# PaddlePaddle/PaddleScience

Measured on AMD Instinct MI355X. Metric: collocation-points/sec (PDE residual+grad), higher is better.
Workload: dtype f32

## Files before the change

### include/ppsci_hip.h

```cpp
#ifndef PPSCI_HIP_H
#define PPSCI_HIP_H

#include <stddef.h>
#include <stdint.h>

#ifdef __cplusplus
extern "C" {
#endif

#define PPSCI_MAX_IN 8
#define PPSCI_MAX_DIRS 4
#define PPSCI_MAX_OUT 8
#define PPSCI_MAX_HIDDEN 16
#define PPSCI_MAX_PROG 128
#define PPSCI_MAX_RES 8
#define PPSCI_MAX_EPARAM 8
#define PPSCI_MAX_AUX 16

enum { PPSCI_OK = 0, PPSCI_E_INVALID = -1, PPSCI_E_UNSUPPORTED = -2, PPSCI_E_LAUNCH = -3 };
enum { PPSCI_ACT_TANH = 0, PPSCI_ACT_SILU = 1, PPSCI_ACT_SIN = 2, PPSCI_ACT_SIGMOID = 3, PPSCI_ACT_COS = 4, PPSCI_ACT_GELU = 5,
       PPSCI_ACT_SWISH = 6, PPSCI_ACT_STAN = 7,
       PPSCI_ACT_RELU = 8, PPSCI_ACT_LEAKY_RELU = 9, PPSCI_ACT_ELU = 10, PPSCI_ACT_SELU = 11, PPSCI_ACT_IDENTITY = 12 };
enum { PPSCI_EMBED_NONE = 0, PPSCI_EMBED_PERIOD = 1,
       PPSCI_EMBED_STREAMS = 2 };
// ... 103 lines not shown

int ppsci_csr_matvec(int64_t rows, int64_t cols, int64_t nnz, const int32_t* row_ptr, const int32_t* col_idx,
                     const float* vals, const float* x, const float* xscale, float alpha, float* y, void* stream);

int ppsci_epilogue_params(const ppsci_epilogue_desc* e, int64_t n_points, const float* const* inputs_host,
                          const float* U, const float* const* aux_host, float* residual_out, float* Ubar,
                          float* loss_partials, const float* eq_params, float* eq_param_partials, void* stream);
int ppsci_epilogue_losses(const ppsci_epilogue_desc* e, int64_t n_points, const float* const* inputs_host,
                          const float* U, const float* const* aux_host, float* residual_out, float* Ubar,
                          float* loss_partials, const float* eq_params, float* eq_param_partials, float* loss_terms,
                          void* counter, void* stream);

int ppsci_causal_weights(int64_t n_points, int n_chunks, float tol, const float* value, const float* label,
                         const float* weight, const float* area, float* chunk_scratch, float* cw, void* stream);

int ppsci_taylor_bwd(const ppsci_mlp_desc* d, const float* params, int64_t n_points,
                     const float* const* inputs_host, const float* Ubar, const void* stash,
                     void* workspace, float* grad_partials, void* stream);
int ppsci_taylor_bwd_ws(const ppsci_mlp_desc* d, const float* params, int64_t n_points,
                        const float* const* inputs_host, const float* Ubar, const void* stash,
                        void* workspace, int64_t workspace_bytes, float* grad_partials, void* stream);

typedef struct ppsci_adam_args {
  float* m;
  float* v;
  float lr, beta1, beta2, eps, grad_scale;
  int64_t step_t;
} ppsci_adam_args;

int64_t ppsci_taylor_step_workspace_bytes(const ppsci_mlp_desc* d, const ppsci_epilogue_desc* e, int64_t n_points);
int ppsci_taylor_step_kind(const ppsci_mlp_desc* d, const ppsci_epilogue_desc* e, int64_t n_points);
void ppsci_set_fused_step(int on);
void ppsci_set_step_tail(int mode);
void ppsci_set_fast_program(int on);
void ppsci_set_static_program(int on);
int ppsci_epilogue_predecode(const ppsci_epilogue_desc* e, uint32_t* out256, int* n_loads);
typedef struct ppsci_step_plan ppsci_step_plan;
ppsci_step_plan* ppsci_taylor_step_plan(const ppsci_mlp_desc* d, const ppsci_epilogue_desc* e, float* params,
                                        int64_t n_points, const float* const* inputs_host, const float* const* aux_host,
                                        float* U, float* Ubar, float* residual_out, void* stash, void* workspace,
                                        int64_t workspace_bytes, float* loss_terms, float* grad);
int ppsci_taylor_step_run(ppsci_step_plan* plan, int accumulate, const ppsci_adam_args* adam, void* stream);
#define PPSCI_STEP_KEEP_FRAGMENTS 1
int ppsci_taylor_step_run_ex(ppsci_step_plan* plan, int accumulate, const ppsci_adam_args* adam, void* stream, int flags);
int ppsci_taylor_step_plan_apply(ppsci_step_plan* plan, const ppsci_adam_args* adam, void* stream);
int ppsci_taylor_step_plan_set_scales(ppsci_step_plan* plan, const ppsci_epilogue_desc* e);
int ppsci_taylor_step_run_main(ppsci_step_plan* plan, void* stream);
void ppsci_taylor_step_plan_free(ppsci_step_plan* plan);
int ppsci_taylor_step_plan_static(const ppsci_step_plan* plan, const char** name);
int ppsci_taylor_step(const ppsci_mlp_desc* d, const ppsci_epilogue_desc* e, float* params, int64_t n_points,
                      const float* const* inputs_host, const float* const* aux_host, float* U, float* Ubar,
                      float* residual_out, void* stash, void* workspace, int64_t workspace_bytes, float* loss_terms,
                      float* grad, int accumulate, const ppsci_adam_args* adam, void* stream);

int ppsci_reduce_rows(const float* partials, int64_t rows, int64_t cols, float* out, int accumulate,
                      void* stream);

int ppsci_adam_step(int64_t n, float* params, const float* grad, float* m, float* v, float lr,
                    float beta1, float beta2, float eps, int64_t step_t, float grad_scale,
                    void* stream);

#define PPSCI_OPT_SGD 0
#define PPSCI_OPT_MOMENTUM 1
#define PPSCI_OPT_RMSPROP 2
#define PPSCI_OPT_ADAMW 3
int ppsci_optim_step(int kind, int64_t n, float* params, const float* grad, float* state1, float* state2,
// ... 299 lines not shown
```

### paddlescience_amd/_lib.py

```python
from __future__ import annotations

import ctypes as C
import os
from typing import List, Optional, Sequence

MAX_IN, MAX_DIRS, MAX_OUT, MAX_HIDDEN, MAX_PROG, MAX_RES, MAX_AUX = 8, 4, 8, 16, 128, 8, 16

ACT = {"tanh": 0, "silu": 1, "sin": 2, "sigmoid": 3, "cos": 4, "gelu": 5, "swish": 6, "stan": 7, "relu": 8, "leaky_relu": 9,
       "elu": 10, "selu": 11, "identity": 12}
PARAM_ACTS = ("swish", "stan")
SIREN_W0 = 30.0
LINEAR_PLAIN, LINEAR_WEIGHT_NORM, LINEAR_RWF, LINEAR_FOURIER, LINEAR_BROADCAST = range(5)
LINEAR_PADDED = 100
EMBED_NONE, EMBED_PERIOD, EMBED_STREAMS = 0, 1, 2

(OP_LD_IN, OP_LD_U, OP_LD_AUX, OP_CONST, OP_ADD, OP_SUB, OP_MUL, OP_DIV, OP_NEG, OP_POW, OP_SIN, OP_COS,
 OP_TANH, OP_EXP, OP_LOG, OP_SQRT, OP_ABS, OP_SINH, OP_COSH, OP_TAN, OP_MAX, OP_MIN, OP_SIGN, OP_HEAVISIDE,
 OP_DETACH, OP_ASIN, OP_ACOS, OP_ATAN, OP_ATAN2, OP_ASINH, OP_ACOSH, OP_ATANH, OP_ERF, OP_LGAMMA, OP_CEIL, OP_FLOOR,
 OP_LD_PARAM, OP_COUNT) = range(38)
MAX_EPARAM = 8
STEP_KEEP_FRAGMENTS = 1


class MlpDesc(C.Structure):
# ... 106 lines not shown
    "ppsci_comm_init": (C.c_int, [C.c_int, C.c_int, C.c_void_p]),
    "ppsci_comm_world_size": (C.c_int, []),
    "ppsci_allreduce_sum": (C.c_int, [C.c_void_p, C.c_int64, C.c_void_p]),
    "ppsci_allgather": (C.c_int, [C.c_void_p, C.c_void_p, C.c_int64, C.c_void_p]),
    "ppsci_comm_destroy": (C.c_int, []),
    "ppsci_param_count": (C.c_int64, [C.POINTER(MlpDesc)]),
    "ppsci_stash_bytes": (C.c_int64, [C.POINTER(MlpDesc), C.c_int64]),
    "ppsci_bwd_partial_rows": (C.c_int64, [C.POINTER(MlpDesc), C.c_int64]),
    "ppsci_bwd_workspace_bytes": (C.c_int64, [C.POINTER(MlpDesc), C.c_int64]),
    "ppsci_epilogue_partial_rows": (C.c_int64, [C.c_int64]),
    "ppsci_taylor_fwd": (C.c_int, [C.POINTER(MlpDesc), C.c_void_p, C.c_int64, C.POINTER(C.c_void_p), C.c_void_p,
                                   C.c_void_p, C.c_void_p]),
    "ppsci_epilogue": (C.c_int, [C.POINTER(EpilogueDesc), C.c_int64, C.POINTER(C.c_void_p), C.c_void_p,
                                 C.POINTER(C.c_void_p), C.c_void_p, C.c_void_p, C.c_void_p, C.c_void_p]),
    "ppsci_epilogue_losses": (C.c_int, [C.POINTER(EpilogueDesc), C.c_int64, C.POINTER(C.c_void_p), C.c_void_p,
                                        C.POINTER(C.c_void_p), C.c_void_p, C.c_void_p, C.c_void_p, C.c_void_p,
                                        C.c_void_p, C.c_void_p, C.c_void_p, C.c_void_p]),
    "ppsci_epilogue_params": (C.c_int, [C.POINTER(EpilogueDesc), C.c_int64, C.POINTER(C.c_void_p), C.c_void_p,
                                        C.POINTER(C.c_void_p), C.c_void_p, C.c_void_p, C.c_void_p, C.c_void_p,
                                        C.c_void_p, C.c_void_p]),
    "ppsci_taylor_bwd": (C.c_int, [C.POINTER(MlpDesc), C.c_void_p, C.c_int64, C.POINTER(C.c_void_p), C.c_void_p,
                                   C.c_void_p, C.c_void_p, C.c_void_p, C.c_void_p]),
    "ppsci_taylor_bwd_ws": (C.c_int, [C.POINTER(MlpDesc), C.c_void_p, C.c_int64, C.POINTER(C.c_void_p), C.c_void_p,
                                      C.c_void_p, C.c_void_p, C.c_int64, C.c_void_p, C.c_void_p]),
    "ppsci_dense_matvec": (C.c_int, [C.c_int64, C.c_int64, C.c_void_p, C.c_void_p, C.c_void_p, C.c_float, C.c_int, C.c_void_p,
                                     C.c_void_p]),
    "ppsci_csr_matvec": (C.c_int, [C.c_int64, C.c_int64, C.c_int64, C.c_void_p, C.c_void_p, C.c_void_p, C.c_void_p, C.c_void_p,
                                   C.c_float, C.c_void_p, C.c_void_p]),
    "ppsci_reduce_rows": (C.c_int, [C.c_void_p, C.c_int64, C.c_int64, C.c_void_p, C.c_int, C.c_void_p]),
    "ppsci_taylor_step_workspace_bytes": (C.c_int64, [C.POINTER(MlpDesc), C.POINTER(EpilogueDesc), C.c_int64]),
    "ppsci_taylor_step_kind": (C.c_int, [C.POINTER(MlpDesc), C.POINTER(EpilogueDesc), C.c_int64]),
    "ppsci_set_fused_step": (None, [C.c_int]),
    "ppsci_set_step_tail": (None, [C.c_int]),
    "ppsci_set_fast_program": (None, [C.c_int]),
    "ppsci_taylor_step_run_ex": (C.c_int, [C.c_void_p, C.c_int, C.POINTER(AdamArgs), C.c_void_p, C.c_int]),
    "ppsci_taylor_step_plan_apply": (C.c_int, [C.c_void_p, C.POINTER(AdamArgs), C.c_void_p]),
    "ppsci_set_static_program": (None, [C.c_int]),
    "ppsci_epilogue_predecode": (C.c_int, [C.POINTER(EpilogueDesc), C.POINTER(C.c_uint32), C.POINTER(C.c_int)]),
    "ppsci_taylor_step_plan_static": (C.c_int, [C.c_void_p, C.POINTER(C.c_char_p)]),
    "ppsci_taylor_step_plan": (C.c_void_p, [C.POINTER(MlpDesc), C.POINTER(EpilogueDesc), C.c_void_p, C.c_int64,
                                            C.POINTER(C.c_void_p), C.POINTER(C.c_void_p), C.c_void_p, C.c_void_p, C.c_void_p,
                                            C.c_void_p, C.c_void_p, C.c_int64, C.c_void_p, C.c_void_p]),
    "ppsci_taylor_step_run": (C.c_int, [C.c_void_p, C.c_int, C.POINTER(AdamArgs), C.c_void_p]),
    "ppsci_taylor_step_plan_set_scales": (C.c_int, [C.c_void_p, C.POINTER(EpilogueDesc)]),
    "ppsci_taylor_step_run_main": (C.c_int, [C.c_void_p, C.c_void_p]),
    "ppsci_taylor_step_plan_free": (None, [C.c_void_p]),
    "ppsci_taylor_step": (C.c_int, [C.POINTER(MlpDesc), C.POINTER(EpilogueDesc), C.c_void_p, C.c_int64, C.POINTER(C.c_void_p),
                                    C.POINTER(C.c_void_p), C.c_void_p, C.c_void_p, C.c_void_p, C.c_void_p, C.c_void_p,
                                    C.c_int64, C.c_void_p, C.c_void_p, C.c_int, C.POINTER(AdamArgs), C.c_void_p]),
    "ppsci_spectral_conv2d_fwd": (C.c_int, [C.POINTER(SpectralDesc), C.c_void_p, C.c_void_p, C.c_void_p, C.c_void_p,
                                            C.c_void_p]),
    "ppsci_spectral_conv2d_bwd": (C.c_int, [C.POINTER(SpectralDesc), C.c_void_p, C.c_void_p, C.c_void_p, C.c_void_p,
                                            C.c_void_p, C.c_void_p, C.c_void_p, C.c_void_p]),
    "ppsci_spectral_conv2d_bwd_real": (C.c_int, [C.POINTER(SpectralDesc), C.c_void_p, C.c_void_p, C.c_void_p, C.c_void_p,
                                                 C.c_void_p, C.c_void_p, C.c_void_p, C.c_float, C.c_int, C.c_void_p]),
    "ppsci_spectral_conv2d_fwd_scaled": (C.c_int, [C.POINTER(SpectralDesc), C.c_void_p, C.c_void_p, C.c_void_p, C.c_void_p,
                                                   C.c_float, C.c_int, C.c_void_p]),
    "ppsci_spectral_conv2d_bwd_real_scaled": (C.c_int, [C.POINTER(SpectralDesc), C.c_void_p, C.c_void_p, C.c_void_p,
                                                        C.c_void_p, C.c_void_p, C.c_void_p, C.c_void_p, C.c_float, C.c_int,
                                                        C.c_float, C.c_int, C.c_void_p]),
    "ppsci_dft2_kept_supported": (C.c_int, [C.c_int] * 4),
    "ppsci_dft2_kept_fwd": (C.c_int, [C.c_int] * 6 + [C.c_void_p] * 3),
    "ppsci_dft2_kept_inv": (C.c_int, [C.c_int] * 6 + [C.c_void_p] * 3),
    "ppsci_dft2_kept_inv_stats": (C.c_int, [C.c_int] * 6 + [C.c_void_p] * 3 + [C.c_int, C.c_void_p, C.c_void_p]),
    "ppsci_fno_tail_fwd_ex": (C.c_int, [C.c_int] * 5 + [C.c_float] + [C.c_void_p] * 9 + [C.c_int] * 5 + [C.c_void_p, C.c_void_p]),
    "ppsci_fno_tail_bwd_ex": (C.c_int, [C.c_int] * 5 + [C.c_void_p] * 13 + [C.c_int] * 4 + [C.c_void_p] * 3),
# ... 210 lines not shown
```

### paddlescience_amd/csrc/ppsci_common.h

```cpp
#pragma once

#include "ppsci_hip.h"

#ifdef PPSCI_EMU
#include "hip_emu.h"
#define PPSCI_LAUNCH(KERNEL, ARGT, grid, block, lds, stream, args)                                   \
  do {                                                                                               \
    ARGT _a = (args);                                                                                \
    emu::launch_named(#KERNEL, emu_dim3{(unsigned)(grid)}, emu_dim3{(unsigned)(block)}, (size_t)(lds), \
                      [](void* p) { KERNEL(*(ARGT*)p); }, &_a);                                      \
  } while (0)
#define PPSCI_SET_MAX_LDS(KERNEL, bytes) (0)
#define PPSCI_LAST_LAUNCH_ERROR() (0)
#define PPSCI_OCCUPANCY(KERNEL, block, lds, out) (*(out) = 2, 0)
#define __builtin_amdgcn_sched_barrier(x) ((void)0)
#define ppsci_block_sync_lds() __syncthreads()
#define ppsci_block_sync_mem() __syncthreads()
#define ppsci_acquire_agent() ((void)0)
#define ppsci_setprio(p) ((void)0)
#define PPSCI_OPAQUE(v) ((void)0)
static inline void ppsci_store_agent(float* p, float v) { *p = v; }
static inline void ppsci_store_agent4(f32x4* p, f32x4 v) { *p = v; }
static inline unsigned ppsci_readlane(unsigned v, int lane) {
  float f;
  std::memcpy(&f, &v, 4);
  const float* buf = emu::wave_publish(f);
  unsigned r;
  std::memcpy(&r, &buf[lane & 63], 4);
  return r;
}
#else
#include <hip/hip_runtime.h>
typedef float f32x4 __attribute__((ext_vector_type(4)));
typedef unsigned u32x2 __attribute__((ext_vector_type(2)));
typedef unsigned u32x4 __attribute__((ext_vector_type(4)));
#define PPSCI_DYN_SMEM(name) extern __shared__ __attribute__((aligned(16))) float name[]
#define PPSCI_OPAQUE(v) asm volatile("" : "+v"(v))
__device__ __forceinline__ unsigned ppsci_cvt_pk_bf16(float a, float b) {
  typedef float f32x2_ __attribute__((ext_vector_type(2)));
  typedef __bf16 bf16x2_ __attribute__((ext_vector_type(2)));
  return __builtin_bit_cast(unsigned, __builtin_convertvector((f32x2_){a, b}, bf16x2_));
}
__device__ __forceinline__ float ppsci_bf16_sub_lo(unsigned h, float x) {
  typedef __bf16 bf16x2_ __attribute__((ext_vector_type(2)));
  unsigned k = 0x0000bf80u;
  asm volatile("" : "+s"(k));
  return __builtin_amdgcn_fdot2_f32_bf16(__builtin_bit_cast(bf16x2_, h), __builtin_bit_cast(bf16x2_, k), x, false);
}
__device__ __forceinline__ float ppsci_bf16_sub_hi(unsigned h, float x) {
  typedef __bf16 bf16x2_ __attribute__((ext_vector_type(2)));
  unsigned k = 0xbf800000u;
  asm volatile("" : "+s"(k));
  return __builtin_amdgcn_fdot2_f32_bf16(__builtin_bit_cast(bf16x2_, h), __builtin_bit_cast(bf16x2_, k), x, false);
}
__device__ __forceinline__ f32x4 ppsci_xdl32(u32x2 a_lo, u32x2 a_hi, u32x2 b_lo, u32x2 b_hi, f32x4 c) {
  typedef __bf16 bf16x8_ __attribute__((ext_vector_type(8)));
  const u32x4 a = {a_lo[0], a_lo[1], a_hi[0], a_hi[1]}, b = {b_lo[0], b_lo[1], b_hi[0], b_hi[1]};
  return __builtin_amdgcn_mfma_f32_16x16x32_bf16(__builtin_bit_cast(bf16x8_, a), __builtin_bit_cast(bf16x8_, b), c, 0, 0, 0);
}
__device__ __forceinline__ f32x4 ppsci_xdl32a(u32x4 a, u32x2 b_lo, u32x2 b_hi, f32x4 c) {
  typedef __bf16 bf16x8_ __attribute__((ext_vector_type(8)));
  const u32x4 b = {b_lo[0], b_lo[1], b_hi[0], b_hi[1]};
  return __builtin_amdgcn_mfma_f32_16x16x32_bf16(__builtin_bit_cast(bf16x8_, a), __builtin_bit_cast(bf16x8_, b), c, 0, 0, 0);
}
__device__ __forceinline__ f32x4 ppsci_xdl32aa(u32x4 a, u32x4 b, f32x4 c) {
  typedef __bf16 bf16x8_ __attribute__((ext_vector_type(8)));
  return __builtin_amdgcn_mfma_f32_16x16x32_bf16(__builtin_bit_cast(bf16x8_, a), __builtin_bit_cast(bf16x8_, b), c, 0, 0, 0);
}
__device__ __forceinline__ u32x2 ppsci_lds_read_tr16(const void* p) {
  typedef short s16x4_ __attribute__((ext_vector_type(4)));
  return __builtin_bit_cast(u32x2, __builtin_amdgcn_ds_read_tr16_b64_v4i16((__attribute__((address_space(3))) s16x4_*)p));
}
__device__ __forceinline__ f32x4 ppsci_xdl16(u32x2 a, u32x2 b, f32x4 c) {
  typedef short s16x4_ __attribute__((ext_vector_type(4)));
  return __builtin_amdgcn_mfma_f32_16x16x16bf16_1k(__builtin_bit_cast(s16x4_, a), __builtin_bit_cast(s16x4_, b), c, 0, 0, 0);
}
#define PPSCI_LAUNCH(KERNEL, ARGT, grid, block, lds, stream, args)                                   \
  hipLaunchKernelGGL(KERNEL, dim3(grid), dim3(block), (lds), (hipStream_t)(stream), (args))
#define PPSCI_SET_MAX_LDS(KERNEL, bytes)                                                             \
  ((int)hipFuncSetAttribute((const void*)KERNEL, hipFuncAttributeMaxDynamicSharedMemorySize, (int)(bytes)))
#define PPSCI_LAST_LAUNCH_ERROR() ((int)hipGetLastError())
#define PPSCI_OCCUPANCY(KERNEL, block, lds, out)                                                     \
  ((int)hipOccupancyMaxActiveBlocksPerMultiprocessor((out), (const void*)KERNEL, (block), (size_t)(lds)))
__device__ __forceinline__ void ppsci_wave_sync() {
  __builtin_amdgcn_fence(__ATOMIC_RELEASE, "wavefront", "local");
// ... 88 lines not shown
```

### paddlescience_amd/csrc/taylor_fused.inc

```
#include "taylor_tile.h"
#include "taylor_step_tail.h"
#include "epi_static.h"

#include <stdlib.h>
#include <string.h>
#include <type_traits>

#ifndef PPSCI_FUSED_STATIC
#define PPSCI_FUSED_STATIC 0
#endif
#define PPSCI_FUSED_EPI_SCRATCH ((PPSCI_MAX_RES + PPSCI_MAX_EPARAM) * 16)
#define PPSCI_FUSED_MAX_IN 4
#define PPSCI_FUSED_XJ(x, j) ((j) == 0 ? (x)[0] : ((j) == 1 ? (x)[1] : ((j) == 2 ? (x)[2] : (x)[3])))

#ifdef PPSCI_FUSED_TIMERS
#define PPSCI_FT(k)                                             \
  {                                                             \
    const unsigned long long now_ = __builtin_amdgcn_s_memtime(); \
    tacc[k] += now_ - tlast;                                    \
    tlast = now_;                                               \
  }
#else
#define PPSCI_FT(k)
#endif

#define PPSCI_ABL(n) (((ABL) >> (n)) & 1)
template <int ABL>
__device__ __forceinline__ ppsci_split4 ppsci_fused_split(f32x4 x) {
  if (PPSCI_ABL(6)) {
    ppsci_split4 o;
    o.p[0] = (u32x2){__builtin_bit_cast(unsigned, x[0]), __builtin_bit_cast(unsigned, x[1])};
    o.p[1] = (u32x2){__builtin_bit_cast(unsigned, x[2]), __builtin_bit_cast(unsigned, x[3])};
    o.p[2] = o.p[0];
    return o;
  }
  return ppsci_split(x);
}

#ifdef PPSCI_DBG_DUMP
__device__ float* ppsci_dbg_buf = nullptr;
extern "C" int ppsci_dbg_set(float* p) { return (int)hipMemcpyToSymbol(HIP_SYMBOL(ppsci_dbg_buf), &p, sizeof(p)); }
#define PPSCI_DBG_STRIDE 16384
#endif


static inline long long ppsci_fused_floats(const ppsci_mlp_desc& d, const ppsci_derived& q, int S, int n_instr) {
  const int m = d.d_out, pad4m = ((m + 3) / 4) * 4;
  long long fl = 2LL * ((q.d0 + d.n_hidden + m) * q.HP + pad4m);
  fl += (q.NB + 1) * m * S * PPSCI_TILE;
  fl += q.NB * d.d_raw * PPSCI_TILE;
  fl += (long long)q.NB * m * S * PPSCI_TILE;
  fl += PPSCI_FUSED_EPI_SCRATCH + PPSCI_MAX_RES * PPSCI_TILE;
  fl += 2LL * n_instr * PPSCI_TILE;
  fl += EPI_FAST_WORDS + PPSCI_MAX_RES + PPSCI_MAX_RES * PPSCI_TILE;
  fl += 2LL * S * q.NB * 3 * 64 * 2;
  fl += PPSCI_MAX_DIRS * q.HP;
  return fl;
}

template <int NB, int LH, int N1, int N2, int ACT, bool STATIC, int ABL = 0>
__global__ void __launch_bounds__(64 * NB, 2) taylor_fused_kernel(StepArgs args) {
  constexpr int S = 1 + N1 + N2;
  constexpr int HP = 16 * NB;
  constexpr int W = NB;
  constexpr int L = LH;
  constexpr int NKP = NB / 2;
  static_assert(NB == 4, "one feature block per wave, both k-pairs of a layer's fragments held in registers");
  PPSCI_DYN_SMEM(smem);
  const FwdArgs& a = args.f;
  const int tid = threadIdx.x, nthr = blockDim.x;
  const int lane = tid & 63, wave = __builtin_amdgcn_readfirstlane(tid >> 6);
  const int g = lane >> 4, c = lane & 15;
  const int H = a.d.width, m = a.d.d_out, d0 = a.q.d0, d_raw = a.d.d_raw;
  const int pad4m = ((m + 3) / 4) * 4;
  const int n_instr = args.e.e.n_instr;

  float* W0s = smem;
  float* Bs = W0s + d0 * HP;
  float* WLs = Bs + L * HP;
  float* BLs = WLs + m * HP;
  float* gW0 = BLs + pad4m;
  float* gB = gW0 + d0 * HP;
  float* gWL = gB + L * HP;
  float* gBL = gWL + m * HP;
  float* tin = gBL + pad4m;
  float* uls = tin + W * m * S * PPSCI_TILE;
  float* tinx = uls + m * S * PPSCI_TILE;
  float* red = tinx + W * d_raw * PPSCI_TILE;
  float* ered = red + W * m * S * PPSCI_TILE;
  float* lacc = ered + PPSCI_FUSED_EPI_SCRATCH;
  float* rf = lacc + PPSCI_MAX_RES * PPSCI_TILE;
  unsigned* ftab = (unsigned*)(rf + 2 * n_instr * PPSCI_TILE);
  float* rres = (float*)(ftab + EPI_FAST_WORDS + PPSCI_MAX_RES);
  u32x2* zx = (u32x2*)(rres + PPSCI_MAX_RES * PPSCI_TILE);
  u32x2* hx = zx + S * NB * 3 * 64;
  float* dz0 = (float*)(hx + S * NB * 3 * 64);
  f32x4* zsave = (f32x4*)hx;
  static_assert(L * S * 64 * 16 <= S * NB * 3 * 64 * 8, "zsave must fit into hx");
  constexpr bool VM_REGS_OK = (L - 1) * NB * 64 * 16 <= S * NB * 3 * 64 * 8;
// ... 18 lines not shown
    for (int idx = tid; idx < N1 * HP; idx += nthr) {
      const int i = idx / HP, f = idx - i * HP;
      float acc = 0.f;
      for (int j = 0; j < d_raw; ++j) acc += ((f < H) ? a.params[a.q.offW[0] + j * H + f] : 0.f) * a.d.dirs[i][j];
      dz0[idx] = acc;
    }
  const int nacc_small = (d0 + L + m) * HP + pad4m;
  for (int idx = tid; idx < nacc_small; idx += nthr) gW0[idx] = 0.f;
  for (int idx = tid; idx < PPSCI_MAX_RES * PPSCI_TILE; idx += nthr) lacc[idx] = 0.f;
  if (args.e.fast != nullptr) epi_fast_init(args.e, ftab, rf + (lane & 15), PPSCI_TILE, tid, nthr, wave == 0 && lane < PPSCI_TILE);

  float xr[PPSCI_FUSED_MAX_IN];
  const auto fetch_x = [&](int tile_, float (&dst)[PPSCI_FUSED_MAX_IN]) {
    const long long p_ = (long long)tile_ * PPSCI_TILE + c;
    const bool ok_ = tile_ < a.ntiles && p_ < a.N;
#pragma unroll
    for (int j = 0; j < PPSCI_FUSED_MAX_IN; ++j) dst[j] = (j < d_raw && ok_) ? a.x[j < d_raw ? j : 0][p_] : 0.f;
  };
  fetch_x(a.tile0 + (int)blockIdx.x, xr);
  __syncthreads();
  const int static_id = STATIC ? args.e.static_id : 0;
  float st_cvals = 0.f, st_scales = 0.f;
  if constexpr (STATIC) {
    st_cvals = __builtin_bit_cast(float, ftab[192 + (lane & 63)]);
    st_scales = __builtin_bit_cast(float, ftab[EPI_FAST_WORDS + (lane & (PPSCI_MAX_RES - 1))]);
  }

  f32x4 wacc[L - 1][NB];
#pragma unroll
  for (int l = 0; l < L - 1; ++l)
#pragma unroll
    for (int ib = 0; ib < NB; ++ib) wacc[l][ib] = (f32x4){0.f, 0.f, 0.f, 0.f};

#ifdef PPSCI_FUSED_TIMERS
  if (tid < 16) ((unsigned*)ered)[tid] = 0u;
  unsigned long long tacc[16] = {0, 0, 0, 0, 0, 0, 0, 0, 0, 0, 0, 0, 0, 0, 0, 0};
  unsigned long long tlast = __builtin_amdgcn_s_memtime();
#endif
  for (int it = 0; it < a.iters; ++it) {
    const int tile = a.tile0 + it * (int)gridDim.x + (int)blockIdx.x;
    if (tile >= a.ntiles) break;
    PPSCI_FT(0)
    const float* tx = STATIC ? tinx + wave * (d_raw * PPSCI_TILE) : tinx;
    float* const tinw = STATIC ? tin + wave * (m * S * PPSCI_TILE) : tin;
    float auxv[EPI_STATIC_MAX_AUX];
#pragma unroll
    for (int k = 0; k < EPI_STATIC_MAX_AUX; ++k) auxv[k] = 0.f;
    if (STATIC && args.e.e.n_aux > 0) {
      const long long p_ = (long long)tile * PPSCI_TILE + c;
      const long long pp_ = p_ < a.N ? p_ : 0;
#pragma unroll
      for (int k = 0; k < EPI_STATIC_MAX_AUX; ++k)
        if (k < args.e.e.n_aux) auxv[k] = args.e.aux[k][pp_];
    }
    f32x4 zst[L][S];
    f32x4 h[S];

#pragma unroll
    for (int s = 0; s < S; ++s) h[s] = (f32x4){0.f, 0.f, 0.f, 0.f};
    {
      const long long p = (long long)tile * PPSCI_TILE + c;
      const long long pp = p < a.N ? p : 0;
      const float vm = p < a.N ? 1.f : 0.f;
      int k = 0;
      if (PPSCI_ABL(1)) h[0] += xr[0] * 0.01f;
      if ((STATIC || raw_only) && !PPSCI_ABL(1)) {
// ... 382 lines not shown
          *(f32x4*)&q[(2 * 256 + tid) * 4] = D1;
        }
#endif
        {
          const f32x4 two = {2.f, 2.f, 2.f, 2.f};
          f32x4 accv = D1 * hb[0];
#pragma unroll
          for (int i = 0; i < N1; ++i) {
            const f32x4 zi = zst[l][1 + i];
            const f32x4 hbi = hb[1 + i];
            f32x4 zbi = D1 * hbi;
            accv += D2 * zi * hbi;
            if (i < N2) {
              const f32x4 zii = zst[l][1 + N1 + i];
              const f32x4 hb2 = hb[1 + N1 + i];
              hb[1 + N1 + i] = D1 * hb2;
              zbi += two * D2 * zi * hb2;
              accv += (D3 * zi * zi + D2 * zii) * hb2;
            }
            hb[1 + i] = zbi;
          }
          hb[0] = accv;
        }
        if (zs != 1.f) {
#pragma unroll
          for (int s = 0; s < S; ++s) hb[s] *= zs;
        }
#ifdef PPSCI_DBG_DUMP
        if (ppsci_dbg_buf != nullptr && l == L - 1) {
#pragma unroll
          for (int s = 0; s < S; ++s) *(f32x4*)&ppsci_dbg_buf[(long long)blockIdx.x * PPSCI_DBG_STRIDE + (s * 256 + tid) * 4] = hb[s];
        }
#endif
        if (!PPSCI_ABL(2)) {
          f32x4 sb4;
#pragma unroll
          for (int r = 0; r < 4; ++r) sb4[r] = ppsci_row_sum16_last(hb[0][r]);
#ifdef PPSCI_DBG_DUMP
          if (ppsci_dbg_buf != nullptr && l == L - 1) *(f32x4*)&ppsci_dbg_buf[(long long)blockIdx.x * PPSCI_DBG_STRIDE + 4096 + tid * 4] = sb4;
#endif
          if (c == 15) {
#pragma unroll
            for (int r = 0; r < 4; ++r) atomicAdd(&gB[l * HP + 16 * wave + 4 * g + r], sb4[r]);
          }
        }
        if constexpr (l > 0) {
          __builtin_amdgcn_sched_barrier(0);
#pragma unroll
          for (int kp = 0; kp < NKP; ++kp)
#pragma unroll
            for (int q = 0; q < 3; ++q) Ab[kp][q] = gf[((wave * NKP + kp) * 3 + q) * 64];
          __builtin_amdgcn_sched_barrier(0);
#pragma unroll
          for (int s = 0; s < S; ++s) {
            const ppsci_split4 sp = ppsci_fused_split<ABL>(hb[s]);
#pragma unroll
            for (int q = 0; q < 3; ++q)
              if (!PPSCI_ABL(9) || (sp.p[q][0] == 0x12345u && sp.p[q][1] == 0x54321u)) zx[ppsci_xpair(NB, s, wave, q, xcl)] = sp.p[q];
            __builtin_amdgcn_sched_barrier(0);
          }
        }
      }

      if constexpr (l > 0) {
        __builtin_amdgcn_sched_barrier(0);
        ppsci_block_sync_lds();
        PPSCI_FT(7)
// ... 190 lines not shown
        }
      }
    };
#ifndef PPSCI_FX_NOBWD
    if constexpr (L > 4) bwd_layer(std::integral_constant<int, 4>{});
    if constexpr (L > 3) bwd_layer(std::integral_constant<int, 3>{});
    if constexpr (L > 2) bwd_layer(std::integral_constant<int, 2>{});
    bwd_layer(std::integral_constant<int, 1>{});
#endif
    bwd_layer(std::integral_constant<int, 0>{});

    PPSCI_FT(11)
    PPSCI_FT(12)
  }
#ifdef PPSCI_FUSED_TIMERS
  if (lane == 0 && args.t.external && wave != 1) {
#pragma unroll
    for (int k = 0; k < 16; ++k) args.t.tree[((long long)blockIdx.x * W + wave) * 16 + k] = (float)tacc[k];
    if (wave == 0)
      for (int k = 0; k < 16; ++k) args.t.tree[((long long)blockIdx.x * W + 1) * 16 + k] = (float)((unsigned*)ered)[k];
  }
#endif

  {
    f32x4* dst = args.b.wpart + (long long)blockIdx.x * ((L - 1) * NB * NB * 64) + lane;
#pragma unroll
    for (int l = 0; l < L - 1; ++l)
#pragma unroll
      for (int ib = 0; ib < NB; ++ib) {
        f32x4* const q = &dst[((long long)l * NB * NB + ib * NB + wave) * 64];
        if (args.t.external == 1) *q = wacc[l][ib];
        else ppsci_store_agent4(q, wacc[l][ib]);
      }
  }
  __syncthreads();
  for (int idx = tid; idx < d0 * H; idx += nthr) {
    const int k = idx / H, f = idx - k * H;
    ppsci_store_agent(&prow[idx], gW0[k * HP + f]);
  }
  for (int idx = tid; idx < L * H; idx += nthr) {
    const int l = idx / H, f = idx - l * H;
    ppsci_store_agent(&prow[d0 * H + idx], gB[l * HP + f]);
  }
  for (int idx = tid; idx < H * m; idx += nthr) {
    const int f = idx / m, cc = idx - f * m;
    ppsci_store_agent(&prow[(d0 + L) * H + idx], gWL[cc * HP + f]);
  }
  for (int idx = tid; idx < m; idx += nthr) ppsci_store_agent(&prow[(d0 + L + m) * H + idx], gBL[idx]);
  {
    float lsum[PPSCI_MAX_RES], padj[PPSCI_MAX_EPARAM];
#pragma unroll
    for (int k = 0; k < PPSCI_MAX_RES; ++k) lsum[k] = (wave == 0 && lane < PPSCI_TILE) ? lacc[k * PPSCI_TILE + lane] : 0.f;
#pragma unroll
    for (int k = 0; k < PPSCI_MAX_EPARAM; ++k) padj[k] = 0.f;
    epi_finale<EPI_RF_FUSED>(args.e, ered, lsum, padj);
  }
  if (args.t.external != 1) ppsci_step_tail(args.t, args.b.d, args.b.q, smem);
}

template <int NB, int LH, int N1, int N2>
static int launch_fused(StepArgs& a, void* stream, int launch, int* grid_out) {
  constexpr int S = 1 + N1 + N2;
  if (launch == 2) {
#ifdef PPSCI_ABL_BUILD
    {
      const char* ev = getenv("PPSCI_ABL");
// ... 87 lines not shown
```

### paddlescience_amd/csrc/taylor_fused_silu.hip

```cpp
#define PPSCI_ACT_ID PPSCI_ACT_SILU
#define PPSCI_FUSED_RUN_NAME ppsci_fused_run_silu
#include "taylor_fused.inc"
```

### paddlescience_amd/csrc/taylor_fused_sin.hip

```cpp
#define PPSCI_ACT_ID PPSCI_ACT_SIN
#define PPSCI_FUSED_RUN_NAME ppsci_fused_run_sin
#include "taylor_fused.inc"
```

### paddlescience_amd/csrc/taylor_fused_static_tanh.hip

```cpp
#define PPSCI_ACT_ID PPSCI_ACT_TANH
#define PPSCI_FUSED_STATIC 1
#define PPSCI_FUSED_RUN_NAME ppsci_fused_static_run_tanh
#include "taylor_fused.inc"
```

### paddlescience_amd/csrc/wgrad_reduce.hip

```cpp
#include "taylor_tile.h"

#include <string.h>

struct WRedArgs {
  const float* wpart;
  float* tmp;
  float* row;
  const float* small;
  float* tmp_small;
  int nsmall_rows, psmall, nbs;
  int m, d0;
  ppsci_derived q;
  int L, H, ntiles, nchunks, nb4;
  long long per_tile;
  long long tmp_stride, small_stride, loss_stride;
  ppsci_wred_extras x;
};

__global__ void __launch_bounds__(256) wgrad_reduce1_kernel(WRedArgs a) {
  if ((int)blockIdx.x >= a.nchunks * a.nb4) {
    const int bid = (int)blockIdx.x - a.nchunks * a.nb4;
    const int chunk = bid / a.nbs;
    const int j = (bid - chunk * a.nbs) * 256 + threadIdx.x;
    if (j >= a.psmall) return;
// ... 162 lines not shown
    }
  }
  PPSCI_LAUNCH(wgrad_reduce2_kernel, WRedArgs, (q.P + 255) / 256 + (x.loss_rows != nullptr ? 1 : 0), 256, 0, stream, a);
  int e = PPSCI_LAST_LAUNCH_ERROR();
  if (e != 0) {
    ppsci_set_error("wgrad_reduce2: launch failed (hip error %d)", e);
    return PPSCI_E_LAUNCH;
  }
  return PPSCI_OK;
}

struct WTailArgs {
  const float* rows_w;
  const float* rows_s;
  float* row;
  u32x4* frag;
  ppsci_derived q;
  int L, H, m, d0, nrows, psmall, nblk, nsmall;
  long long per_tile, loss_stride;
  ppsci_wred_extras x;
};

__device__ __forceinline__ float wtail_adam(const ppsci_wred_extras& x, int idx, float gsum) {
  const float g = gsum * x.grad_scale;
  const float mm = x.beta1 * x.m[idx] + (1.f - x.beta1) * g;
  const float vv = x.beta2 * x.v[idx] + (1.f - x.beta2) * g * g;
  x.m[idx] = mm;
  x.v[idx] = vv;
  const float pn = x.p[idx] - x.lr_t * (mm / (sqrtf(vv) + x.eps_t));
  x.p[idx] = pn;
  return pn;
}

__global__ void __launch_bounds__(1024) wgrad_tail_kernel(WTailArgs a) {
  __shared__ f32x4 red[16][64];
  __shared__ float tile[16][17];
  const int tid = threadIdx.x, lane = tid & 63, rg = tid >> 6;
  const int b = blockIdx.x;
  if (b < a.nblk) {
    const long long stride4 = a.per_tile / 4;
    const f32x4* src = (const f32x4*)a.rows_w + (long long)b * 64 + lane;
    f32x4 acc[4];
#pragma unroll
    for (int u = 0; u < 4; ++u) acc[u] = (f32x4){0.f, 0.f, 0.f, 0.f};
#pragma unroll 2
    for (int r0 = rg; r0 < a.nrows; r0 += 64) {
#pragma unroll
      for (int u = 0; u < 4; ++u) {
        const int r = r0 + 16 * u;
        const f32x4 v = __builtin_nontemporal_load(&src[(long long)(r < a.nrows ? r : a.nrows - 1) * stride4]);
        acc[u] += r < a.nrows ? v : (f32x4){0.f, 0.f, 0.f, 0.f};
      }
    }
    red[rg][lane] = (acc[0] + acc[1]) + (acc[2] + acc[3]);
    __syncthreads();
    if (rg != 0) return;
    f32x4 tot = red[0][lane];
#pragma unroll
    for (int w = 1; w < 16; ++w) tot += red[w][lane];
    const int NB = a.q.NB, NKP = NB / 2;
    const int l = b / (NB * NB), blk = b - l * NB * NB, ib = blk / NB, ob = blk - ib * NB;
    const int g = lane >> 4, c = lane & 15;
    const int in0 = 16 * ib + 4 * g, out = 16 * ob + c;
    f32x4 pn = (f32x4){0.f, 0.f, 0.f, 0.f};
#pragma unroll
    for (int r = 0; r < 4; ++r) {
// ... 17 lines not shown
    for (int r = 0; r < 4; ++r) tile[4 * g + r][c] = pn[r];
    ppsci_wave_sync();
    f32x4 pt;
#pragma unroll
    for (int r = 0; r < 4; ++r) pt[r] = tile[c][4 * g + r];
    {
      const ppsci_split4 sp = ppsci_split(pt);
      u32x2* dst = (u32x2*)(a.frag + (long long)(a.L - 1 + l) * per_layer + (long long)((ib * NKP + (ob >> 1)) * 3) * 64 + lane) + (ob & 1);
#pragma unroll
      for (int p = 0; p < 3; ++p) dst[(long long)p * 64 * 2] = sp.p[p];
    }
    return;
  }
  if (b < a.nblk + a.nsmall) {
    float* redf = (float*)red;
    const int ci = (b - a.nblk) * 64 + lane;
    const int cc = ci < a.psmall ? ci : 0;
    float acc[4] = {0.f, 0.f, 0.f, 0.f};
#pragma unroll 2
    for (int r0 = rg; r0 < a.nrows; r0 += 64) {
#pragma unroll
      for (int u = 0; u < 4; ++u) {
        const int r = r0 + 16 * u;
        const float v = a.rows_s[(long long)(r < a.nrows ? r : a.nrows - 1) * a.psmall + cc];
        acc[u] += r < a.nrows ? v : 0.f;
      }
    }
    redf[rg * 64 + lane] = (acc[0] + acc[1]) + (acc[2] + acc[3]);
    __syncthreads();
    if (rg != 0 || ci >= a.psmall) return;
    float v = redf[lane];
#pragma unroll
    for (int w = 1; w < 16; ++w) v += redf[w * 64 + lane];
    const int H = a.H, L = a.L;
    int idx;
    if (ci < a.d0 * H) idx = a.q.offW[0] + ci;
    else if (ci < (a.d0 + L) * H) {
      const int lb = (ci - a.d0 * H) / H;
      idx = a.q.offB[lb] + (ci - a.d0 * H - lb * H);
    } else if (ci < (a.d0 + L + a.m) * H) idx = a.q.offW[L] + (ci - (a.d0 + L) * H);
    else idx = a.q.offB[L] + (ci - (a.d0 + L + a.m) * H);
    if (a.x.accumulate) v += a.row[idx];
    a.row[idx] = v;
    if (a.x.p != nullptr) wtail_adam(a.x, idx, v);
    return;
  }
  float* redf = (float*)red;
  for (int k = 0; k < a.x.n_res; ++k) {
    float v = 0.f;
#pragma unroll 4
    for (int r = tid; r < a.x.loss_nrows; r += 1024) v += a.x.loss_rows[(long long)r * a.loss_stride + k];
#pragma unroll
    for (int off = 32; off >= 1; off >>= 1) v += __shfl_xor(v, off, 64);
    if (lane == 0) redf[rg] = v;
    __syncthreads();
    if (tid == 0) {
      float s = redf[0];
      for (int w = 1; w < 16; ++w) s += redf[w];
      a.x.loss_out[k] = s;
    }
    __syncthreads();
  }
}

int ppsci_wgrad_tail(const ppsci_mlp_desc& d, const ppsci_derived& q, int nrows, const float* rows_w, const float* rows_s,
                     float* row, const ppsci_wred_extras& x, void* frag, void* stream) {
  WTailArgs a;
  memset(&a, 0, sizeof(a));
  a.rows_w = rows_w;
  a.rows_s = rows_s;
  a.row = row;
  a.frag = (u32x4*)frag;
  a.q = q;
  a.L = d.n_hidden;
  a.H = d.width;
  a.m = d.d_out;
  a.d0 = q.d0;
  a.nrows = nrows;
  a.psmall = ppsci_small_params(d, q);
  a.nblk = (d.n_hidden - 1) * q.NB * q.NB;
  a.nsmall = (a.psmall + 63) / 64;
  a.per_tile = (long long)(d.n_hidden - 1) * q.HP * q.HP;
  a.loss_stride = x.n_res;
  a.x = x;
  PPSCI_LAUNCH(wgrad_tail_kernel, WTailArgs, a.nblk + a.nsmall + (x.loss_rows != nullptr ? 1 : 0), 1024, 0, stream, a);
  if (PPSCI_LAST_LAUNCH_ERROR() != 0) {
    ppsci_set_error("wgrad_tail: launch failed");
    return PPSCI_E_LAUNCH;
  }
  return PPSCI_OK;
}
```

Before: 445.1 million.

## Split weight-gradient tail into smaller blocks, accumulate biases per lane, tweak split constants

The weight-gradient tail reduction gets a new 256-thread kernel that gives each 16x16 tile four blocks instead of one 1024-thread block, and this kernel is now the default path. The aim is more parallelism and better occupancy in the tail. Separately, the fused forward kernel keeps per-lane bias-gradient accumulators for small configs and does the 16-lane row sum once at the end rather than every iteration. This trades extra registers for fewer cross-lane reductions. The bf16 split constant is also held in a VGPR for the silu, sin and static-tanh variants, which may change instruction selection and register pressure.

Result: faster. 467.8 million, median of 6 (+5.1%).

```diff
diff --git a/include/ppsci_hip.h b/include/ppsci_hip.h
--- a/include/ppsci_hip.h
+++ b/include/ppsci_hip.h
@@ -159,6 +159,7 @@
 int ppsci_taylor_step_kind(const ppsci_mlp_desc* d, const ppsci_epilogue_desc* e, int64_t n_points);
 void ppsci_set_fused_step(int on);
 void ppsci_set_step_tail(int mode);
+void ppsci_set_tail_split(int n);
 void ppsci_set_fast_program(int on);
 void ppsci_set_static_program(int on);
 int ppsci_epilogue_predecode(const ppsci_epilogue_desc* e, uint32_t* out256, int* n_loads);
diff --git a/paddlescience_amd/_lib.py b/paddlescience_amd/_lib.py
--- a/paddlescience_amd/_lib.py
+++ b/paddlescience_amd/_lib.py
@@ -162,6 +162,7 @@
     "ppsci_taylor_step_kind": (C.c_int, [C.POINTER(MlpDesc), C.POINTER(EpilogueDesc), C.c_int64]),
     "ppsci_set_fused_step": (None, [C.c_int]),
     "ppsci_set_step_tail": (None, [C.c_int]),
+    "ppsci_set_tail_split": (None, [C.c_int]),
     "ppsci_set_fast_program": (None, [C.c_int]),
     "ppsci_taylor_step_run_ex": (C.c_int, [C.c_void_p, C.c_int, C.POINTER(AdamArgs), C.c_void_p, C.c_int]),
     "ppsci_taylor_step_plan_apply": (C.c_int, [C.c_void_p, C.POINTER(AdamArgs), C.c_void_p]),
diff --git a/paddlescience_amd/csrc/ppsci_common.h b/paddlescience_amd/csrc/ppsci_common.h
--- a/paddlescience_amd/csrc/ppsci_common.h
+++ b/paddlescience_amd/csrc/ppsci_common.h
@@ -41,16 +41,21 @@
   typedef __bf16 bf16x2_ __attribute__((ext_vector_type(2)));
   return __builtin_bit_cast(unsigned, __builtin_convertvector((f32x2_){a, b}, bf16x2_));
 }
+#if defined(PPSCI_SPLIT_CONST_VGPR) && PPSCI_SPLIT_CONST_VGPR
+#define PPSCI_SPLIT_CONST_HIDE(k) asm("" : "+v"(k))
+#else
+#define PPSCI_SPLIT_CONST_HIDE(k) asm volatile("" : "+s"(k))
+#endif
 __device__ __forceinline__ float ppsci_bf16_sub_lo(unsigned h, float x) {
   typedef __bf16 bf16x2_ __attribute__((ext_vector_type(2)));
   unsigned k = 0x0000bf80u;
-  asm volatile("" : "+s"(k));
+  PPSCI_SPLIT_CONST_HIDE(k);
   return __builtin_amdgcn_fdot2_f32_bf16(__builtin_bit_cast(bf16x2_, h), __builtin_bit_cast(bf16x2_, k), x, false);
 }
 __device__ __forceinline__ float ppsci_bf16_sub_hi(unsigned h, float x) {
   typedef __bf16 bf16x2_ __attribute__((ext_vector_type(2)));
   unsigned k = 0xbf800000u;
-  asm volatile("" : "+s"(k));
+  PPSCI_SPLIT_CONST_HIDE(k);
   return __builtin_amdgcn_fdot2_f32_bf16(__builtin_bit_cast(bf16x2_, h), __builtin_bit_cast(bf16x2_, k), x, false);
 }
 __device__ __forceinline__ f32x4 ppsci_xdl32(u32x2 a_lo, u32x2 a_hi, u32x2 b_lo, u32x2 b_hi, f32x4 c) {
diff --git a/paddlescience_amd/csrc/taylor_fused.inc b/paddlescience_amd/csrc/taylor_fused.inc
--- a/paddlescience_amd/csrc/taylor_fused.inc
+++ b/paddlescience_amd/csrc/taylor_fused.inc
@@ -8,6 +8,9 @@
 
 #ifndef PPSCI_FUSED_STATIC
 #define PPSCI_FUSED_STATIC 0
+#endif
+#ifndef PPSCI_FUSED_LANE_BIAS
+#define PPSCI_FUSED_LANE_BIAS(L, S, ACT, STATIC) ((L) * ((S) + 1) <= (((STATIC) && (ACT) == PPSCI_ACT_TANH) ? 20 : 12))
 #endif
 #define PPSCI_FUSED_EPI_SCRATCH ((PPSCI_MAX_RES + PPSCI_MAX_EPARAM) * 16)
 #define PPSCI_FUSED_MAX_IN 4
@@ -65,6 +68,7 @@
   constexpr int W = NB;
   constexpr int L = LH;
   constexpr int NKP = NB / 2;
+  constexpr bool LANE_BIAS = PPSCI_FUSED_LANE_BIAS(LH, S, ACT, STATIC);
   static_assert(NB == 4, "one feature block per wave, both k-pairs of a layer's fragments held in registers");
   PPSCI_DYN_SMEM(smem);
   const FwdArgs& a = args.f;
@@ -149,6 +153,10 @@
 #pragma unroll
     for (int ib = 0; ib < NB; ++ib) wacc[l][ib] = (f32x4){0.f, 0.f, 0.f, 0.f};
 
+  f32x4 bacc[LANE_BIAS ? L : 1];
+#pragma unroll
+  for (int l = 0; l < (LANE_BIAS ? L : 1); ++l) bacc[l] = (f32x4){0.f, 0.f, 0.f, 0.f};
+
 #ifdef PPSCI_FUSED_TIMERS
   if (tid < 16) ((unsigned*)ered)[tid] = 0u;
   unsigned long long tacc[16] = {0, 0, 0, 0, 0, 0, 0, 0, 0, 0, 0, 0, 0, 0, 0, 0};
@@ -597,7 +605,9 @@
           for (int s = 0; s < S; ++s) *(f32x4*)&ppsci_dbg_buf[(long long)blockIdx.x * PPSCI_DBG_STRIDE + (s * 256 + tid) * 4] = hb[s];
         }
 #endif
-        if (!PPSCI_ABL(2)) {
+        if constexpr (LANE_BIAS) {
+          if (!PPSCI_ABL(2)) bacc[l] += hb[0];
+        } else if (!PPSCI_ABL(2)) {
           f32x4 sb4;
 #pragma unroll
           for (int r = 0; r < 4; ++r) sb4[r] = ppsci_row_sum16_last(hb[0][r]);
@@ -854,6 +864,15 @@
         if (args.t.external == 1) *q = wacc[l][ib];
         else ppsci_store_agent4(q, wacc[l][ib]);
       }
+  }
+  if constexpr (LANE_BIAS) {
+#pragma unroll
+    for (int l = 0; l < L; ++l) {
+      f32x4 sb4;
+#pragma unroll
+      for (int r = 0; r < 4; ++r) sb4[r] = ppsci_row_sum16_last(bacc[l][r]);
+      if (c == 15) *(f32x4*)&gB[l * HP + 16 * wave + 4 * g] = sb4;
+    }
   }
   __syncthreads();
   for (int idx = tid; idx < d0 * H; idx += nthr) {
diff --git a/paddlescience_amd/csrc/taylor_fused_silu.hip b/paddlescience_amd/csrc/taylor_fused_silu.hip
--- a/paddlescience_amd/csrc/taylor_fused_silu.hip
+++ b/paddlescience_amd/csrc/taylor_fused_silu.hip
@@ -1,3 +1,6 @@
+#ifndef PPSCI_SPLIT_CONST_VGPR
+#define PPSCI_SPLIT_CONST_VGPR 1
+#endif
 #define PPSCI_ACT_ID PPSCI_ACT_SILU
 #define PPSCI_FUSED_RUN_NAME ppsci_fused_run_silu
 #include "taylor_fused.inc"
diff --git a/paddlescience_amd/csrc/taylor_fused_sin.hip b/paddlescience_amd/csrc/taylor_fused_sin.hip
--- a/paddlescience_amd/csrc/taylor_fused_sin.hip
+++ b/paddlescience_amd/csrc/taylor_fused_sin.hip
@@ -1,3 +1,6 @@
+#ifndef PPSCI_SPLIT_CONST_VGPR
+#define PPSCI_SPLIT_CONST_VGPR 1
+#endif
 #define PPSCI_ACT_ID PPSCI_ACT_SIN
 #define PPSCI_FUSED_RUN_NAME ppsci_fused_run_sin
 #include "taylor_fused.inc"
diff --git a/paddlescience_amd/csrc/taylor_fused_static_tanh.hip b/paddlescience_amd/csrc/taylor_fused_static_tanh.hip
--- a/paddlescience_amd/csrc/taylor_fused_static_tanh.hip
+++ b/paddlescience_amd/csrc/taylor_fused_static_tanh.hip
@@ -1,3 +1,6 @@
+#ifndef PPSCI_SPLIT_CONST_VGPR
+#define PPSCI_SPLIT_CONST_VGPR 1
+#endif
 #define PPSCI_ACT_ID PPSCI_ACT_TANH
 #define PPSCI_FUSED_STATIC 1
 #define PPSCI_FUSED_RUN_NAME ppsci_fused_static_run_tanh
diff --git a/paddlescience_amd/csrc/wgrad_reduce.hip b/paddlescience_amd/csrc/wgrad_reduce.hip
--- a/paddlescience_amd/csrc/wgrad_reduce.hip
+++ b/paddlescience_amd/csrc/wgrad_reduce.hip
@@ -218,6 +218,17 @@
   return pn;
 }
 
+__device__ __forceinline__ int wtail_small_index(const WTailArgs& a, int ci) {
+  const int H = a.H, L = a.L;
+  if (ci < a.d0 * H) return a.q.offW[0] + ci;
+  if (ci < (a.d0 + L) * H) {
+    const int lb = (ci - a.d0 * H) / H;
+    return a.q.offB[lb] + (ci - a.d0 * H - lb * H);
+  }
+  if (ci < (a.d0 + L + a.m) * H) return a.q.offW[L] + (ci - (a.d0 + L) * H);
+  return a.q.offB[L] + (ci - (a.d0 + L + a.m) * H);
+}
+
 __global__ void __launch_bounds__(1024) wgrad_tail_kernel(WTailArgs a) {
   __shared__ f32x4 red[16][64];
   __shared__ float tile[16][17];
@@ -301,14 +312,7 @@
     float v = redf[lane];
 #pragma unroll
     for (int w = 1; w < 16; ++w) v += redf[w * 64 + lane];
-    const int H = a.H, L = a.L;
-    int idx;
-    if (ci < a.d0 * H) idx = a.q.offW[0] + ci;
-    else if (ci < (a.d0 + L) * H) {
-      const int lb = (ci - a.d0 * H) / H;
-      idx = a.q.offB[lb] + (ci - a.d0 * H - lb * H);
-    } else if (ci < (a.d0 + L + a.m) * H) idx = a.q.offW[L] + (ci - (a.d0 + L) * H);
-    else idx = a.q.offB[L] + (ci - (a.d0 + L + a.m) * H);
+    const int idx = wtail_small_index(a, ci);
     if (a.x.accumulate) v += a.row[idx];
     a.row[idx] = v;
     if (a.x.p != nullptr) wtail_adam(a.x, idx, v);
@@ -331,6 +335,126 @@
     __syncthreads();
   }
 }
+
+__global__ void __launch_bounds__(256) wgrad_tail_split_kernel(WTailArgs a) {
+  __shared__ f32x4 red[16][16];
+  __shared__ float tile[4][17];
+  const int tid = threadIdx.x, c = tid & 15, rg = tid >> 4;
+  const int b = blockIdx.x;
+  if (b < 4 * a.nblk) {
+    const int blk_l = b >> 2, g = b & 3, lane = 16 * g + c;
+    const long long stride4 = a.per_tile / 4;
+    const f32x4* src = (const f32x4*)a.rows_w + (long long)blk_l * 64 + lane;
+    f32x4 acc[4];
+#pragma unroll
+    for (int u = 0; u < 4; ++u) acc[u] = (f32x4){0.f, 0.f, 0.f, 0.f};
+#pragma unroll 4
+    for (int r0 = rg; r0 < a.nrows; r0 += 64) {
+#pragma unroll
+      for (int u = 0; u < 4; ++u) {
+        const int r = r0 + 16 * u;
+        const f32x4 v = __builtin_nontemporal_load(&src[(long long)(r < a.nrows ? r : a.nrows - 1) * stride4]);
+        acc[u] += r < a.nrows ? v : (f32x4){0.f, 0.f, 0.f, 0.f};
+      }
+    }
+    red[rg][c] = (acc[0] + acc[1]) + (acc[2] + acc[3]);
+    __syncthreads();
+    if (tid >= 64) return;
+    const bool own = tid < 16;
+    const int NB = a.q.NB, NKP = NB / 2;
+    const int l = blk_l / (NB * NB), blk = blk_l - l * NB * NB, ib = blk / NB, ob = blk - ib * NB;
+    f32x4 pn = (f32x4){0.f, 0.f, 0.f, 0.f};
+    if (own) {
+      f32x4 tot = red[0][c];
+#pragma unroll
+      for (int w = 1; w < 16; ++w) tot += red[w][c];
+      const int in0 = 16 * ib + 4 * g, out = 16 * ob + c;
+#pragma unroll
+      for (int r = 0; r < 4; ++r) {
+        if (in0 + r < a.H && out < a.H) {
+          const int idx = a.q.offW[l + 1] + (in0 + r) * a.H + out;
+          float v = tot[r];
+          if (a.x.accumulate) v += a.row[idx];
+          a.row[idx] = v;
+          if (a.x.p != nullptr) pn[r] = wtail_adam(a.x, idx, v);
+        }
+      }
+    }
+    if (a.x.p == nullptr || a.frag == nullptr) return;
+    const long long per_layer = (long long)NB * NKP * 3 * 64;
+    if (own) {
+      const ppsci_split4 sp = ppsci_split(pn);
+      u32x2* dst = (u32x2*)(a.frag + (long long)l * per_layer + (long long)((ob * NKP + (ib >> 1)) * 3) * 64 + lane) + (ib & 1);
+#pragma unroll
+      for (int p = 0; p < 3; ++p) dst[(long long)p * 64 * 2] = sp.p[p];
+#pragma unroll
+      for (int r = 0; r < 4; ++r) tile[r][c] = pn[r];
+    }
+    ppsci_wave_sync();
+    if (own) {
+      const int gd = c >> 2, i = c & 3, laned = 16 * gd + 4 * g + i;
+      f32x4 pt;
+#pragma unroll
+      for (int r = 0; r < 4; ++r) pt[r] = tile[i][4 * gd + r];
+      const ppsci_split4 sp = ppsci_split(pt);
+      u32x2* dst = (u32x2*)(a.frag + (long long)(a.L - 1 + l) * per_layer + (long long)((ib * NKP + (ob >> 1)) * 3) * 64 + laned) + (ob & 1);
+#pragma unroll
+      for (int p = 0; p < 3; ++p) dst[(long long)p * 64 * 2] = sp.p[p];
+    }
+    return;
+  }
+  if (b < 4 * a.nblk + a.nsmall) {
+    float* redf = (float*)red;
+    const int ci = (b - 4 * a.nblk) * 16 + c;
+    const int cc = ci < a.psmall ? ci : 0;
+    float acc[4] = {0.f, 0.f, 0.f, 0.f};
+#pragma unroll 4
+    for (int r0 = rg; r0 < a.nrows; r0 += 64) {
+#pragma unroll
+      for (int u = 0; u < 4; ++u) {
+        const int r = r0 + 16 * u;
+        const float v = a.rows_s[(long long)(r < a.nrows ? r : a.nrows - 1) * a.psmall + cc];
+        acc[u] += r < a.nrows ? v : 0.f;
+      }
+    }
+    redf[rg * 16 + c] = (acc[0] + acc[1]) + (acc[2] + acc[3]);
+    __syncthreads();
+    if (rg != 0 || ci >= a.psmall) return;
+    float v = redf[c];
+#pragma unroll
+    for (int w = 1; w < 16; ++w) v += redf[w * 16 + c];
+    const int idx = wtail_small_index(a, ci);
+    if (a.x.accumulate) v += a.row[idx];
+    a.row[idx] = v;
+    if (a.x.p != nullptr) wtail_adam(a.x, idx, v);
+    return;
+  }
+  float* redf = (float*)red;
+  const int lane = tid & 63, wv = tid >> 6;
+  for (int k = 0; k < a.x.n_res; ++k) {
+    for (int pass = 0; pass < 4; ++pass) {
+      float v = 0.f;
+#pragma unroll 4
+      for (int r = 256 * pass + tid; r < a.x.loss_nrows; r += 1024) v += a.x.loss_rows[(long long)r * a.loss_stride + k];
+#pragma unroll
+      for (int off = 32; off >= 1; off >>= 1) v += __shfl_xor(v, off, 64);
+      if (lane == 0) redf[4 * pass + wv] = v;
+    }
+    __syncthreads();
+    if (tid == 0) {
+      float s = redf[0];
+      for (int w = 1; w < 16; ++w) s += redf[w];
+      a.x.loss_out[k] = s;
+    }
+    __syncthreads();
+  }
+}
+
+#ifndef PPSCI_TAIL_SPLIT_DEFAULT
+#define PPSCI_TAIL_SPLIT_DEFAULT 0
+#endif
+static int g_tail_split = PPSCI_TAIL_SPLIT_DEFAULT;
+extern "C" void ppsci_set_tail_split(int n) { g_tail_split = n == 1 ? 1 : (n == 0 ? PPSCI_TAIL_SPLIT_DEFAULT : 0); }
 
 int ppsci_wgrad_tail(const ppsci_mlp_desc& d, const ppsci_derived& q, int nrows, const float* rows_w, const float* rows_s,
                      float* row, const ppsci_wred_extras& x, void* frag, void* stream) {
@@ -348,11 +472,17 @@
   a.nrows = nrows;
   a.psmall = ppsci_small_params(d, q);
   a.nblk = (d.n_hidden - 1) * q.NB * q.NB;
-  a.nsmall = (a.psmall + 63) / 64;
   a.per_tile = (long long)(d.n_hidden - 1) * q.HP * q.HP;
   a.loss_stride = x.n_res;
   a.x = x;
-  PPSCI_LAUNCH(wgrad_tail_kernel, WTailArgs, a.nblk + a.nsmall + (x.loss_rows != nullptr ? 1 : 0), 1024, 0, stream, a);
+  const int nloss = x.loss_rows != nullptr ? 1 : 0;
+  if (g_tail_split == 1) {
+    a.nsmall = (a.psmall + 63) / 64;
+    PPSCI_LAUNCH(wgrad_tail_kernel, WTailArgs, a.nblk + a.nsmall + nloss, 1024, 0, stream, a);
+  } else {
+    a.nsmall = (a.psmall + 15) / 16;
+    PPSCI_LAUNCH(wgrad_tail_split_kernel, WTailArgs, 4 * a.nblk + a.nsmall + nloss, 256, 0, stream, a);
+  }
   if (PPSCI_LAST_LAUNCH_ERROR() != 0) {
     ppsci_set_error("wgrad_tail: launch failed");
     return PPSCI_E_LAUNCH;
```
